# SamsungLabs/fcaf3d

Measured on AMD Instinct MI355X. Metric: scenes/sec fwd+bwd, ScanNet 100k-pt 2cm voxels, 1/2/4/8 MI355X, higher is better.
Workload: dtype f32

## Files before the change

fcaf3d_amd/csrc/conv.hip:

```cpp
#include "fc_common.h"
#include "../../include/fcaf3d_hip.h"
#ifdef FC_TRACE
__device__ unsigned long long* g_trace_buf_lds;
__device__ int g_trace_cap_lds;
extern "C" int fc_debug_trace_lds(unsigned long long* buf, int cap) {
  FC_HIP(hipMemcpyToSymbol(HIP_SYMBOL(g_trace_buf_lds), &buf, sizeof(buf)));
  FC_HIP(hipMemcpyToSymbol(HIP_SYMBOL(g_trace_cap_lds), &cap, sizeof(cap)));
  return FC_OK;
}
#define TR_BUF g_trace_buf_lds
#define TR_CAP g_trace_cap_lds
#endif
#include "fc_trace.h"

typedef float f32x16 __attribute__((ext_vector_type(16)));
typedef float f32x2 __attribute__((ext_vector_type(2)));
typedef float f32x4 __attribute__((ext_vector_type(4)));

__device__ __attribute__((aligned(16))) float g_zero_row[64];

__device__ int g_fc_prio;
extern "C" int fc_debug_set_prio(int mode) {
  FC_HIP(hipMemcpyToSymbol(HIP_SYMBOL(g_fc_prio), &mode, sizeof(mode)));
  return FC_OK;
// ... 33 lines not shown

__global__ __launch_bounds__(256) void k_amax(const f32x4* __restrict__ x, int64_t n4, const float* __restrict__ tail, int ntail,
                                              unsigned* __restrict__ slot) {
  __shared__ unsigned wm[4];
  __shared__ int last_s;
  unsigned m = 0u;
  const int64_t stride = (int64_t)gridDim.x * 256;
  for (int64_t i = (int64_t)blockIdx.x * 256 + threadIdx.x; i < n4; i += 4 * stride) {
    f32x4 v[4];
#pragma unroll
    for (int q = 0; q < 4; ++q) v[q] = i + q * stride < n4 ? x[i + q * stride] : f32x4{0.f, 0.f, 0.f, 0.f};
#pragma unroll
    for (int q = 0; q < 4; ++q)
#pragma unroll
      for (int j = 0; j < 4; ++j) { const unsigned u = __float_as_uint(v[q][j]) & 0x7fffffffu; m = (u > m && u < 0x7f800000u) ? u : m; }
  }
  if (blockIdx.x == 0 && (int)threadIdx.x < ntail) { const unsigned u = __float_as_uint(tail[threadIdx.x]) & 0x7fffffffu; m = (u > m && u < 0x7f800000u) ? u : m; }
#pragma unroll
  for (int off = 32; off > 0; off >>= 1) { const unsigned o = (unsigned)__shfl_xor((int)m, off, 64); m = o > m ? o : m; }
  if ((threadIdx.x & 63) == 0) wm[threadIdx.x >> 6] = m;
  __syncthreads();
  if (threadIdx.x == 0) {
    unsigned b = wm[0];
    for (int w = 1; w < 4; ++w) b = wm[w] > b ? wm[w] : b;
    if (b > __hip_atomic_load(&slot[1], __ATOMIC_RELAXED, __HIP_MEMORY_SCOPE_AGENT)) atomicMax(&slot[1], b);
    __threadfence();
    last_s = atomicAdd(&slot[2], 1u) == gridDim.x - 1;
    if (last_s) {
      __threadfence();
      slot[0] = atomicExch(&slot[1], 0u);
      slot[2] = 0u;
    }
  }
}

constexpr int AMAX_RING = 2048;
static unsigned* g_amax_ring[16] = {};
static unsigned g_amax_next[16] = {};
static std::mutex g_amax_ring_mu;
static int amax_ring_slot(unsigned** slot) {
  int dev = 0;
  FC_HIP(hipGetDevice(&dev));
  if (dev < 0 || dev >= 16) return FC_EINVAL;
  std::lock_guard<std::mutex> lock(g_amax_ring_mu);
  if (!g_amax_ring[dev]) {
    FC_HIP(hipMalloc((void**)&g_amax_ring[dev], (size_t)AMAX_RING * FC_AMAX_SLOT_BYTES));
    FC_HIP(hipMemset(g_amax_ring[dev], 0, (size_t)AMAX_RING * FC_AMAX_SLOT_BYTES));
  }
  const unsigned i = __atomic_fetch_add(&g_amax_next[dev], 1u, __ATOMIC_RELAXED) % AMAX_RING;
  *slot = g_amax_ring[dev] + (size_t)i * (FC_AMAX_SLOT_BYTES / 4);
  return FC_OK;
}
static int amax_launch(const float* x, int64_t n, unsigned* slot, hipStream_t stream) {
  if (n <= 0) { FC_HIP(hipMemsetAsync(slot, 0, 4, stream)); return FC_OK; }
  const int64_t n4 = n / 4;
  int64_t blocks = fc_cdiv(n4 > 0 ? n4 : 1, 256 * 8);
  if (blocks > 1024) blocks = 1024;
  k_amax<<<(unsigned)blocks, 256, 0, stream>>>(reinterpret_cast<const f32x4*>(x), n4, x + 4 * n4, (int)(n - 4 * n4), slot);
  FC_CHECK_LAUNCH();
  return FC_OK;
}
static thread_local const unsigned* t_amax_hint[2] = {nullptr, nullptr};
struct AmaxHintScope { ~AmaxHintScope() { t_amax_hint[0] = t_amax_hint[1] = nullptr; } };
static int operand_amax(const float* x, int64_t n, int which, hipStream_t stream, const unsigned** out) {
  const unsigned* h = t_amax_hint[which];
  if (h) { *out = h; return FC_OK; }
  unsigned* slot;
  int rc = amax_ring_slot(&slot);
  if (rc) return rc;
  rc = amax_launch(x, n, slot, stream);
  *out = slot;
  return rc;
}
extern "C" int fc_amax(const float* x, int64_t n, unsigned* slot, hipStream_t stream) {
  if (!slot || n < 0 || (n > 0 && !x) || ((uintptr_t)x & 15)) return FC_EINVAL;
  return amax_launch(x, n, slot, stream);
}
extern "C" int fc_conv_amax_hint(const unsigned* amax_in, const unsigned* amax_gout) {
  t_amax_hint[0] = amax_in;
  t_amax_hint[1] = amax_gout;
  return FC_OK;
}

__global__ void k_sum_parts(const float* __restrict__ part, float* __restrict__ out, int64_t elems4, int S) {
  int64_t i = (int64_t)blockIdx.x * blockDim.x + threadIdx.x;
  if (i >= elems4) return;
  float4 a = reinterpret_cast<const float4*>(part)[i];
  for (int s = 1; s < S; ++s) {
    float4 b = reinterpret_cast<const float4*>(part)[(int64_t)s * elems4 + i];
    a.x += b.x; a.y += b.y; a.z += b.z; a.w += b.w;
  }
  reinterpret_cast<float4*>(out)[i] = a;
}

__global__ void k_sum_pairs(const float* __restrict__ part, const int* __restrict__ pos, float* __restrict__ out,
                            int64_t n_out, int K, int Cout) {
  const int c4n = Cout / 4;
  int64_t t = (int64_t)blockIdx.x * blockDim.x + threadIdx.x;
  if (t >= n_out * c4n) return;
  int64_t o = t / c4n;
  int c4 = (int)(t % c4n);
  f32x4 a = {0.f, 0.f, 0.f, 0.f};
  for (int k0 = 0; k0 < K; k0 += 9) {
    int j[9];
#pragma unroll
    for (int u = 0; u < 9; ++u) j[u] = k0 + u < K ? pos[(int64_t)(k0 + u) * n_out + o] : -1;
    f32x4 v[9];
#pragma unroll
    for (int u = 0; u < 9; ++u) {
      const float* src = j[u] >= 0 ? part + ((int64_t)(k0 + u) * n_out + j[u]) * Cout + c4 * 4 : g_zero_row + (c4 & 15) * 4;
      v[u] = *reinterpret_cast<const f32x4*>(src);
    }
#pragma unroll
    for (int u = 0; u < 9; ++u)
      if (j[u] >= 0) a += v[u];
  }
  *reinterpret_cast<f32x4*>(out + o * Cout + c4 * 4) = a;
}

__host__ __device__ static inline int fc_stat_rb(int64_t n) { return n <= 1024 ? 16 : (n <= 4096 ? 64 : 32); }

__device__ __forceinline__ void stat_block_reduce(f32x4 a1, f32x4 a2, float* __restrict__ stats, int C, f32x4* sm ) {
  const int lane = threadIdx.x & 15, rl = threadIdx.x >> 4;
  sm[(rl * 2 + 0) * 16 + lane] = a1;
  sm[(rl * 2 + 1) * 16 + lane] = a2;
  __syncthreads();
  if (rl < 2) {
    f32x4 t = {0.f, 0.f, 0.f, 0.f};
#pragma unroll
    for (int q = 0; q < 16; ++q) t += sm[(q * 2 + rl) * 16 + lane];
    *reinterpret_cast<f32x4*>(stats + ((int64_t)blockIdx.x * 2 + rl) * C + blockIdx.y * 64 + lane * 4) = t;
  }
}

struct StatCh { f32x4 mu, is, ga, be; bool bwd, from_y, has_add; int act; };
__device__ __forceinline__ StatCh stat_channels(const X6Epi& epi, int c) {
  StatCh p;
  p.bwd = epi.bn_x != nullptr;
  p.act = epi.act;
  p.from_y = p.bwd && epi.bn_y != nullptr && epi.act != 0;
  p.has_add = p.bwd && epi.add != nullptr;
  p.mu = f32x4{0.f, 0.f, 0.f, 0.f}; p.is = f32x4{1.f, 1.f, 1.f, 1.f}; p.ga = p.is; p.be = p.mu;
  if (p.bwd) {
    p.mu = *reinterpret_cast<const f32x4*>(epi.mean + c);
    const f32x4 va = *reinterpret_cast<const f32x4*>(epi.var + c);
#pragma unroll
    for (int j = 0; j < 4; ++j) p.is[j] = 1.f / sqrtf(va[j] + epi.eps);
    if (epi.gamma) p.ga = *reinterpret_cast<const f32x4*>(epi.gamma + c);
    if (epi.beta) p.be = *reinterpret_cast<const f32x4*>(epi.beta + c);
  }
  return p;
}
__device__ __forceinline__ void stat_accumulate(const StatCh& p, const X6Epi& epi, const f32x4& a, int64_t at, f32x4& a1, f32x4& a2) {
  f32x4 xv = {0.f, 0.f, 0.f, 0.f}, av = xv, yv = xv;
  if (p.bwd) xv = *reinterpret_cast<const f32x4*>(epi.bn_x + at);
  if (p.has_add) av = *reinterpret_cast<const f32x4*>(epi.add + at);
  if (p.from_y) yv = *reinterpret_cast<const f32x4*>(epi.bn_y + at);
#pragma unroll
  for (int j = 0; j < 4; ++j) {
    float t1, t2;
    x6_epi_terms(p.bwd, p.bwd ? av[j] + a[j] : a[j], xv[j], p.mu[j], p.is[j], p.ga[j], p.be[j], p.act, p.from_y, yv[j], t1, t2);
    a1[j] += t1;
    a2[j] += t2;
  }
}

__global__ __launch_bounds__(256) void k_sum_parts_stats(const float* __restrict__ part, float* __restrict__ out, int64_t n, int C, int S,
                                                         int RB, X6Epi epi) {
  __shared__ f32x4 sm[16 * 2 * 16];
  const int lane = threadIdx.x & 15, rl = threadIdx.x >> 4;
  const int64_t r0 = (int64_t)blockIdx.x * RB;
  const int c = blockIdx.y * 64 + lane * 4;
  const StatCh p = stat_channels(epi, c);
  f32x4 a1 = {0.f, 0.f, 0.f, 0.f}, a2 = a1;
  for (int64_t r = r0 + rl; r < r0 + RB && r < n; r += 16) {
    f32x4 a = *reinterpret_cast<const f32x4*>(part + r * C + c);
    for (int z = 1; z < S; ++z) a += *reinterpret_cast<const f32x4*>(part + ((int64_t)z * n + r) * C + c);
    *reinterpret_cast<f32x4*>(out + r * C + c) = a;
    stat_accumulate(p, epi, a, r * C + c, a1, a2);
  }
  stat_block_reduce(a1, a2, epi.stats, C, sm);
}

__global__ __launch_bounds__(256) void k_sum_pairs_stats(const float* __restrict__ part, const int* __restrict__ pos, float* __restrict__ out,
                                                         int64_t n_out, int K, int Cout, int RB, X6Epi epi) {
  __shared__ f32x4 sm[16 * 2 * 16];
  const int lane = threadIdx.x & 15, rl = threadIdx.x >> 4;
  const int64_t r0 = (int64_t)blockIdx.x * RB;
  const int c = blockIdx.y * 64 + lane * 4;
  const StatCh p = stat_channels(epi, c);
  f32x4 a1 = {0.f, 0.f, 0.f, 0.f}, a2 = a1;
  const int64_t rend = (r0 + RB < n_out) ? r0 + RB : n_out;
  for (int64_t o = r0 + rl; o < rend; o += 32) {
    const int64_t o2 = o + 16;
    const bool two = o2 < rend;
    f32x4 a = {0.f, 0.f, 0.f, 0.f}, b = a;
    for (int k0 = 0; k0 < K; k0 += 9) {
      int j[9], j2[9];
#pragma unroll
      for (int u = 0; u < 9; ++u) {
        j[u] = k0 + u < K ? pos[(int64_t)(k0 + u) * n_out + o] : -1;
        j2[u] = (two && k0 + u < K) ? pos[(int64_t)(k0 + u) * n_out + o2] : -1;
      }
      f32x4 v[9], v2[9];
#pragma unroll
      for (int u = 0; u < 9; ++u) {
        const float* src = j[u] >= 0 ? part + ((int64_t)(k0 + u) * n_out + j[u]) * Cout + c : g_zero_row + lane * 4;
        const float* src2 = j2[u] >= 0 ? part + ((int64_t)(k0 + u) * n_out + j2[u]) * Cout + c : g_zero_row + lane * 4;
        v[u] = *reinterpret_cast<const f32x4*>(src);
        v2[u] = *reinterpret_cast<const f32x4*>(src2);
      }
#pragma unroll
      for (int u = 0; u < 9; ++u) {
        if (j[u] >= 0) a += v[u];
        if (j2[u] >= 0) b += v2[u];
      }
    }
    *reinterpret_cast<f32x4*>(out + o * Cout + c) = a;
    stat_accumulate(p, epi, a, o * Cout + c, a1, a2);
    if (two) {
      *reinterpret_cast<f32x4*>(out + o2 * Cout + c) = b;
      stat_accumulate(p, epi, b, o2 * Cout + c, a1, a2);
    }
  }
  stat_block_reduce(a1, a2, epi.stats, Cout, sm);
}

static_assert(STEM_CIN == 3 && STEM_COUT == 64 && BK == 32, "conv_route.h spells these shapes out");

struct ConvArgs {
  const float *in, *W; const int *nbr, *out_index, *cnt; float* dst;
  int64_t n_rows; int K, Cin, Cout; X6Epi epi; hipStream_t stream;
};
#define FC_LAUNCH(...) __VA_ARGS__<<<grid, 256, 0, a.stream>>>(a.in, a.W, a.nbr, a.out_index, a.cnt, a.dst, a.n_rows, a.K, a.Cin, a.Cout)
#define FC_LAUNCH_EPI(...) __VA_ARGS__<<<grid, 256, 0, a.stream>>>(a.in, a.W, a.nbr, a.out_index, a.cnt, a.dst, a.n_rows, a.K, a.Cin, a.Cout, a.epi)

template <int BM, int BN, int WM>
static void launch_conv_fp32(const ConvRoute& r, const ConvArgs& a, dim3 grid) {
#define FC_LAUNCH_MFMA(KERNEL)                                                                                              \
  do { if (r.wsrc == FC_WSRC_FP32_T) FC_LAUNCH(KERNEL<BM, BN, 32, true, WM, true>); else if (a.nbr) FC_LAUNCH(KERNEL<BM, BN, 32, true, WM>); \
       else FC_LAUNCH(KERNEL<BM, BN, 32, false, WM>); } while (0)
  if (r.family == FC_FAM_MFMA) FC_LAUNCH_MFMA(k_conv_mfma);
  if constexpr (BM >= 128) {
    if (r.family == FC_FAM_MFMA_P) FC_LAUNCH_MFMA(k_conv_mfma_p);
    if (r.family == FC_FAM_GLDS) { if (a.nbr) FC_LAUNCH(k_conv_glds<BM, BN, true, WM>); else FC_LAUNCH(k_conv_glds<BM, BN, false, WM>); }
  }
#undef FC_LAUNCH_MFMA
}

template <int BM, int BN, int WM>
static void launch_conv_x6(const ConvRoute& r, const ConvArgs& a, dim3 grid) {
  if (r.family == FC_FAM_H3R) {
    if constexpr (BM == 128) {
      if (r.buf) FC_LAUNCH_EPI(k_conv_h3r<BN, true, true>);
      else if (a.nbr) FC_LAUNCH_EPI(k_conv_h3r<BN, true, false>);
      else FC_LAUNCH_EPI(k_conv_h3r<BN, false, false>);
    }
  } else if (r.wsrc == FC_WSRC_FP32_T) FC_LAUNCH_EPI(k_conv_x6<BM, BN, true, WM, 1>);
  else if (r.wsrc == FC_WSRC_FP32) { if (a.nbr) FC_LAUNCH_EPI(k_conv_x6<BM, BN, true, WM, 0>); else FC_LAUNCH_EPI(k_conv_x6<BM, BN, false, WM, 0>); }
  else if (r.mode == FC_MODE_BF16 || r.buf) {
    if constexpr (BM == 128) {
      if (r.mode == FC_MODE_BF16) { if (a.nbr) FC_LAUNCH_EPI(k_conv_x6<128, BN, true, 2, 2, 1>); else FC_LAUNCH_EPI(k_conv_x6<128, BN, false, 2, 2, 1>); }
      else if (r.mode == FC_MODE_H3) FC_LAUNCH_EPI(k_conv_x6<128, BN, true, 2, 2, 2, true>);
      else FC_LAUNCH_EPI(k_conv_x6<128, BN, true, 2, 2, 0, true>);
    }
  } else if (r.mode == FC_MODE_H3) { if (a.nbr) FC_LAUNCH_EPI(k_conv_x6<BM, BN, true, WM, 2, 2>); else FC_LAUNCH_EPI(k_conv_x6<BM, BN, false, WM, 2, 2>); }
  else { if (a.nbr) FC_LAUNCH_EPI(k_conv_x6<BM, BN, true, WM, 2>); else FC_LAUNCH_EPI(k_conv_x6<BM, BN, false, WM, 2>); }
}

static int launch_conv(const ConvRoute& r, const ConvArgs& a) {
  const dim3 grid(r.grid[0], r.grid[1], r.grid[2]);
  if (r.family == FC_FAM_STEM) {
    const size_t smem = (size_t)(STEM_ROWS * STEM_FWD_LDA + 96 * 64) * sizeof(float);
    k_stem_fwd<<<(unsigned)fc_cdiv(a.n_rows, STEM_ROWS), 256, smem, a.stream>>>(a.in, a.W, a.nbr, a.dst, nullptr, a.n_rows, a.K);
  } else if (r.family == FC_FAM_FMA) {
    k_conv_fma<<<(unsigned)fc_cdiv(a.n_rows * a.Cout, 256), 256, 0, a.stream>>>(a.in, a.W, a.nbr, a.dst, a.n_rows, a.K, a.Cin, a.Cout, r.wsrc == FC_WSRC_FP32_T ? 1 : 0);
  } else {
#define FC_TILE(BM, BN, WM) do { if (r.family >= FC_FAM_X6) launch_conv_x6<BM, BN, WM>(r, a, grid); else launch_conv_fp32<BM, BN, WM>(r, a, grid); } while (0)
    if (r.bm == 256) FC_TILE(256, 64, 4);
    else if (r.bm == 128 && r.bn == 128) FC_TILE(128, 128, 2);
    else if (r.bm == 128) FC_TILE(128, 64, 2);
    else if (r.bn == 128) launch_conv_fp32<64, 128, 2>(r, a, grid);
    else launch_conv_fp32<64, 64, 2>(r, a, grid);
#undef FC_TILE
  }
  FC_CHECK_LAUNCH();
  return FC_OK;
}
#undef FC_LAUNCH
#undef FC_LAUNCH_EPI

extern "C" {

int fc_conv_fwd_route(int64_t n_in, int64_t n_out, int K, int Cin, int Cout, int flags, int table_kind, int64_t live_tiles, int* out) {
  if (!out || n_in < 0 || n_out < 0 || K < 1 || Cin < 1 || Cout < 1) return FC_EINVAL;
  const ConvRoute r = conv_route({n_in, n_out, K, Cin, Cout}, flags, table_kind, live_tiles, route_env());
  const int f[16] = {r.family, r.bm, r.bn, r.wm, r.S, r.wsrc, r.mode, r.buf, r.epi, (int)r.grid[0], (int)r.grid[1], (int)r.grid[2]};
  for (int i = 0; i < 16; ++i) out[i] = f[i];
  return r.family == FC_FAM_INVALID ? FC_EINVAL : FC_OK;
}

int64_t fc_conv_fwd_ws_bytes(int64_t n_out, int K, int Cin, int Cout, int flags) {
  const ConvRoute r = conv_route({n_out, n_out, K, Cin, Cout}, flags, FC_TABLE_DENSE, 0, route_env());
  return r.S > 1 ? (int64_t)r.S * n_out * Cout * (int64_t)sizeof(float) : 0;
}

int64_t fc_conv_fwd_pairs_ws_bytes(int64_t n_out, int K, int Cout) {
  return (int64_t)K * n_out * Cout * (int64_t)sizeof(float);
}

int64_t fc_conv_stats_blocks(int64_t n_out, int K, int Cin, int Cout, int flags, int pairs) {
  if (n_out < 1) return 0;
  const ConvRoute r = conv_route({n_out, n_out, K, Cin, Cout}, flags, pairs ? FC_TABLE_PAIRS : FC_TABLE_DENSE, 0, route_env());
  if (r.epi == FC_EPI_NONE) return 0;
  return r.epi == FC_EPI_SUM ? fc_cdiv(n_out, fc_stat_rb(n_out)) : fc_cdiv(n_out, r.bm);
}

static int conv_impl(const float* in, const float* W, const int* nbr, const int* out_index, const int* cnt, const int* pos, float* out,
                     int64_t n_in, int64_t n_out, int K, int Cin, int Cout, int64_t live_tiles, int flags, void* ws, int64_t ws_bytes,
                     hipStream_t stream, const X6Epi* epi) {
  AmaxHintScope hint_scope;
  if (n_in < 0 || n_out < 0 || K < 1 || Cin < 1 || Cout < 1) return FC_EINVAL;
  if (n_out == 0 && !cnt) return epi ? FC_EINVAL : FC_OK;
  if (out_index && !nbr) return FC_EINVAL;
  const int table = cnt ? FC_TABLE_PAIRS : out_index ? FC_TABLE_SORTED : nbr ? FC_TABLE_DENSE : FC_TABLE_NONE;
  const ConvRoute r = conv_route({n_in, n_out, K, Cin, Cout}, flags, table | (epi ? FC_TABLE_STATS : 0), live_tiles, route_env());
  if (r.family == FC_FAM_INVALID) return FC_EINVAL;
  if (n_out == 0) return FC_OK;
  ConvArgs a = {in, W, nbr, out_index, cnt, out, n_out, K, Cin, Cout, {}, stream};
  if (r.family == FC_FAM_STEM || r.family == FC_FAM_FMA) return launch_conv(r, a);
  const bool parts = cnt || r.S > 1;
  if (parts && ws_bytes < (int64_t)r.S * n_out * Cout * (int64_t)sizeof(float)) return FC_EWS;
  if (parts) a.dst = (float*)ws;
  if (epi && r.epi == FC_EPI_KERNEL) a.epi = *epi;
  int rc = FC_OK;
  if (r.mode == FC_MODE_H3) rc = operand_amax(in, n_in * (int64_t)Cin, 0, stream, &a.epi.amax_in);
  if (rc == FC_OK) rc = launch_conv(r, a);
  if (rc != FC_OK || !parts) return rc;
  const int rb = fc_stat_rb(n_out);
  const dim3 sgrid((unsigned)fc_cdiv(n_out, rb), Cout / 64);
  if (cnt && epi) k_sum_pairs_stats<<<sgrid, 256, 0, stream>>>(a.dst, pos, out, n_out, K, Cout, rb, *epi);
  else if (cnt) k_sum_pairs<<<(unsigned)fc_cdiv(n_out * (Cout / 4), 256), 256, 0, stream>>>(a.dst, pos, out, n_out, K, Cout);
  else if (epi) k_sum_parts_stats<<<sgrid, 256, 0, stream>>>(a.dst, out, n_out, Cout, r.S, rb, *epi);
  else k_sum_parts<<<(unsigned)fc_cdiv(n_out * Cout / 4, 256), 256, 0, stream>>>(a.dst, out, n_out * Cout / 4, r.S);
  FC_CHECK_LAUNCH();
  return FC_OK;
}

static int conv_pairs_impl(const float* in, const float* W, const int* pair_in, const int* pair_cnt, const int* pair_pos, float* out,
                           int64_t n_in, int64_t n_out, int K, int Cin, int Cout, int64_t live_tiles, int flags, void* ws,
                           int64_t ws_bytes, hipStream_t stream, const X6Epi* epi) {
  if (!pair_in || !pair_cnt || !pair_pos || K > 65535) return FC_EINVAL;
  return conv_impl(in, W, pair_in, nullptr, pair_cnt, pair_pos, out, n_in, n_out, K, Cin, Cout, live_tiles, flags, ws, ws_bytes, stream, epi);
}

static X6Epi stats_epi(float* stats, const float* bn_x = nullptr, const float* mean = nullptr, const float* var = nullptr, const float* gamma = nullptr,
                       const float* beta = nullptr, float eps = 0.f, int act = 0, const float* add = nullptr, const float* bn_y = nullptr) {
  return {stats, bn_x, mean, var, gamma, beta, eps, act, add, bn_y, nullptr};
}

int fc_conv_fwd(const float* in, const float* W, const int* nbr, const int* out_index, float* out, int64_t n_in,
                int64_t n_out, int K, int Cin, int Cout, int flags, void* ws, int64_t ws_bytes, hipStream_t stream) {
  return conv_impl(in, W, nbr, out_index, nullptr, nullptr, out, n_in, n_out, K, Cin, Cout, 0, flags, ws, ws_bytes, stream, nullptr);
}

int fc_conv_fwd_stats(const float* in, const float* W, const int* nbr, const int* out_index, float* out, int64_t n_in,
                      int64_t n_out, int K, int Cin, int Cout, int flags, void* ws, int64_t ws_bytes, float* stats,
                      hipStream_t stream) {
  const X6Epi e = stats_epi(stats);
  return conv_impl(in, W, nbr, out_index, nullptr, nullptr, out, n_in, n_out, K, Cin, Cout, 0, flags, ws, ws_bytes, stream, stats ? &e : nullptr);
}

int fc_conv_fwd_bn_bwd_stats(const float* in, const float* W, const int* nbr, const int* out_index, float* out, int64_t n_in,
                             int64_t n_out, int K, int Cin, int Cout, int flags, void* ws, int64_t ws_bytes, float* stats,
                             const float* bn_x, const float* mean, const float* var, const float* gamma, const float* beta, float eps,
                             int act, const float* add, const float* bn_y, hipStream_t stream) {
  if (!stats || !bn_x || !mean || !var || act < 0 || act > 2) return FC_EINVAL;
  const X6Epi e = stats_epi(stats, bn_x, mean, var, gamma, beta, eps, act, add, bn_y);
  return conv_impl(in, W, nbr, out_index, nullptr, nullptr, out, n_in, n_out, K, Cin, Cout, 0, flags, ws, ws_bytes, stream, &e);
}

int fc_conv_fwd_pairs_tiles(const float* in, const float* W, const int* pair_in, const int* pair_cnt, const int* pair_pos,
                            float* out, int64_t n_in, int64_t n_out, int K, int Cin, int Cout, int64_t live_tiles, int flags,
                            void* ws, int64_t ws_bytes, hipStream_t stream) {
  return conv_pairs_impl(in, W, pair_in, pair_cnt, pair_pos, out, n_in, n_out, K, Cin, Cout, live_tiles, flags, ws, ws_bytes, stream, nullptr);
}

int fc_conv_fwd_pairs_tiles_stats(const float* in, const float* W, const int* pair_in, const int* pair_cnt, const int* pair_pos,
                                  float* out, int64_t n_in, int64_t n_out, int K, int Cin, int Cout, int64_t live_tiles, int flags,
                                  void* ws, int64_t ws_bytes, float* stats, hipStream_t stream) {
  const X6Epi e = stats_epi(stats);
  return conv_pairs_impl(in, W, pair_in, pair_cnt, pair_pos, out, n_in, n_out, K, Cin, Cout, live_tiles, flags, ws, ws_bytes, stream,
                         stats ? &e : nullptr);
}

int fc_conv_fwd_pairs_tiles_bn_bwd_stats(const float* in, const float* W, const int* pair_in, const int* pair_cnt, const int* pair_pos,
                                         float* out, int64_t n_in, int64_t n_out, int K, int Cin, int Cout, int64_t live_tiles, int flags,
                                         void* ws, int64_t ws_bytes, float* stats, const float* bn_x, const float* mean,
                                         const float* var, const float* gamma, const float* beta, float eps, int act,
                                         const float* add, const float* bn_y, hipStream_t stream) {
  if (!stats || !bn_x || !mean || !var || act < 0 || act > 2) return FC_EINVAL;
  const X6Epi e = stats_epi(stats, bn_x, mean, var, gamma, beta, eps, act, add, bn_y);
  return conv_pairs_impl(in, W, pair_in, pair_cnt, pair_pos, out, n_in, n_out, K, Cin, Cout, live_tiles, flags, ws, ws_bytes, stream, &e);
}

int fc_conv_fwd_pairs(const float* in, const float* W, const int* pair_in, const int* pair_cnt, const int* pair_pos,
                      float* out, int64_t n_in, int64_t n_out, int K, int Cin, int Cout, int flags, void* ws,
                      int64_t ws_bytes, hipStream_t stream) {
  return fc_conv_fwd_pairs_tiles(in, W, pair_in, pair_cnt, pair_pos, out, n_in, n_out, K, Cin, Cout, 0, flags, ws, ws_bytes, stream);
}

int64_t fc_x6_weight_image_bytes(int K, int R, int C) { return (int64_t)K * R * C * 6; }

int fc_x6_weight_image(const float* W, void* img, int K, int R, int C, int transposed, hipStream_t stream) {
  if (K < 1 || R < 32 || C < 64 || R % 32 != 0 || C % 64 != 0) return FC_EINVAL;
  const int64_t total = (int64_t)K * (R / 32) * (C / 64) * 256;
  const unsigned nb = (unsigned)fc_cdiv(total, 256);
  if (split_mode() == 2) {
    FC_HIP(hipMemsetAsync((char*)img + 4 * X6_IMG_AMAX_WORD, 0, FC_AMAX_SLOT_BYTES, stream));
    k_x6_weight_image<3><<<nb, 256, 0, stream>>>(W, (u32x4*)img, K, R, C, transposed);
    k_x6_weight_image<2><<<nb, 256, 0, stream>>>(W, (u32x4*)img, K, R, C, transposed);
  } else {
    k_x6_weight_image<0><<<nb, 256, 0, stream>>>(W, (u32x4*)img, K, R, C, transposed);
  }
  FC_CHECK_LAUNCH();
  return FC_OK;
}
// ... 235 lines not shown
```

fcaf3d_amd/csrc/norm_bn.h:

```cpp
#pragma once


__global__ void k_bn1_partial(const float* __restrict__ x, int64_t n, int C, int64_t rpb, float* __restrict__ part) {
  extern __shared__ float sm[];
  const auto [cl, rl, nrl] = lane_coord(C / 4);
  const auto [r0, r1] = row_span(rpb, n);
  const float4 sh = *reinterpret_cast<const float4*>(x + cl * 4);
  float4 a1 = make_float4(0.f, 0.f, 0.f, 0.f), a2 = a1;
  for (int64_t rb = r0 + rl; rb < r1; rb += 4 * (int64_t)nrl) {
    float4 v[4];
#pragma unroll
    for (int u = 0; u < 4; ++u) {
      const int64_t r = rb + (int64_t)u * nrl;
      v[u] = *reinterpret_cast<const float4*>(x + (r < r1 ? r : 0) * C + cl * 4);
    }
#pragma unroll
    for (int u = 0; u < 4; ++u) {
      v[u].x -= sh.x; v[u].y -= sh.y; v[u].z -= sh.z; v[u].w -= sh.w;
      a1.x += v[u].x; a1.y += v[u].y; a1.z += v[u].z; a1.w += v[u].w;
      a2.x += v[u].x * v[u].x; a2.y += v[u].y * v[u].y; a2.z += v[u].z * v[u].z; a2.w += v[u].w * v[u].w;
    }
  }
  *reinterpret_cast<float4*>(&sm[(rl * 2 + 0) * C + cl * 4]) = a1;
  *reinterpret_cast<float4*>(&sm[(rl * 2 + 1) * C + cl * 4]) = a2;
// ... 151 lines not shown
                                unsigned* __restrict__ amax_out) {
  extern __shared__ float sm[];
  const int c0 = blockIdx.y * CG;
  x += c0; gy += c0; gx += c0; mean += c0; var += c0;
  if (y) y += c0;
  if (gy2) gy2 += c0;
  if (gres) gres += c0;
  if (gamma) gamma += c0;
  if (beta) beta += c0;
  const int c4n = CG / 4;
  const int cl = threadIdx.x % c4n, rl = threadIdx.x / c4n;
  const int nrl = blockDim.x / c4n;
  float4 t1, t2;
  bn1_reduce_parts(part, nb, C, cl, rl, nrl, sm, &t1, &t2, CG, c0);
  if (blockIdx.x == 0 && rl == 0) {
    *reinterpret_cast<float4*>(sums + c0 + cl * 4) = t1;
    *reinterpret_cast<float4*>(sums + C + c0 + cl * 4) = t2;
  }
  const float inv_n = 1.f / (float)n;
  float s1[4] = {t1.x * inv_n, t1.y * inv_n, t1.z * inv_n, t1.w * inv_n};
  float s2[4] = {t2.x * inv_n, t2.y * inv_n, t2.z * inv_n, t2.w * inv_n};
  float mu[4], is[4], g[4], bt[4];
#pragma unroll
  for (int j = 0; j < 4; ++j) {
    mu[j] = mean[cl * 4 + j];
    is[j] = 1.f / sqrtf(var[cl * 4 + j] + eps);
    g[j] = gamma ? gamma[cl * 4 + j] : 1.f;
    bt[j] = beta ? beta[cl * 4 + j] : 0.f;
  }
  const bool from_y = act && y;
  const auto [r0, r1] = row_span(rpb, n);
  unsigned am = 0u;
  for (int64_t rb = r0 + rl; rb < r1; rb += 4 * (int64_t)nrl) {
    float xv[4][4], gv[4][4], yv[4][4];
#pragma unroll
    for (int u = 0; u < 4; ++u) {
      const int64_t r = rb + (int64_t)u * nrl;
      const int64_t rc = r < r1 ? r : r0;
      *reinterpret_cast<float4*>(xv[u]) = *reinterpret_cast<const float4*>(x + rc * C + cl * 4);
      *reinterpret_cast<float4*>(gv[u]) = *reinterpret_cast<const float4*>(gy + rc * C + cl * 4);
      if (gy2) {
        const float4 t2 = *reinterpret_cast<const float4*>(gy2 + rc * C + cl * 4);
        gv[u][0] += t2.x; gv[u][1] += t2.y; gv[u][2] += t2.z; gv[u][3] += t2.w;
      }
      if (from_y) *reinterpret_cast<float4*>(yv[u]) = *reinterpret_cast<const float4*>(y + rc * C + cl * 4);
    }
#pragma unroll
    for (int u = 0; u < 4; ++u) {
      const int64_t r = rb + (int64_t)u * nrl;
      if (r >= r1) continue;
      float o[4], gr[4];
#pragma unroll
      for (int j = 0; j < 4; ++j) {
        float gg = gv[u][j];
        if (from_y) gg *= act_bwd_from_y(yv[u][j], act);
        else if (act) gg *= act_bwd_from_pre(bn_pre(xv[u][j], mu[j], is[j], g[j], bt[j]), act);
        float xh = (xv[u][j] - mu[j]) * is[j];
        gr[j] = gg;
        o[j] = g[j] * is[j] * (gg - s1[j] - xh * s2[j]);
      }
      *reinterpret_cast<float4*>(gx + r * C + cl * 4) = *reinterpret_cast<float4*>(o);
      if (gres) *reinterpret_cast<float4*>(gres + r * C + cl * 4) = *reinterpret_cast<float4*>(gr);
#pragma unroll
      for (int j = 0; j < 4; ++j) amax_fold(am, o[j]);
    }
  }
  if (amax_out) amax_commit(am, amax_out);
}

__global__ void k_bn2_apply(const float* __restrict__ x, int64_t n, int C, int64_t rpb, const float* __restrict__ part, int nb, int G,
                            float eps, const float* __restrict__ gamma, const float* __restrict__ beta,
                            const float* __restrict__ residual, int act, float momentum, float* __restrict__ y,
                            float* __restrict__ mean_out, float* __restrict__ var_out, float* __restrict__ cnt_out,
                            float* __restrict__ rmean, float* __restrict__ rvar, long long* __restrict__ nbt, int CG,
                            const int* __restrict__ add_inv, const float* __restrict__ add_src, unsigned* __restrict__ amax_out) {
  extern __shared__ double smd[];
  const int c0 = blockIdx.y * CG;
  x += c0; y += c0; part += c0; mean_out += c0; var_out += c0;
  if (add_src) add_src += c0;
  if (residual) residual += c0;
  if (gamma) gamma += c0;
  if (beta) beta += c0;
  if (rmean) { rmean += c0; rvar += c0; }
  const auto [cl, rl, nrl] = lane_coord(CG / 4);
  double a1[4] = {0., 0., 0., 0.}, a2[4] = {0., 0., 0., 0.};
  const int GC = G * C;
  for (int t = rl; t < nb * G; t += nrl) {
    const int b = t / G, g = t % G;
    const float* src = part + ((int64_t)b * 2) * GC + g * C + cl * 4;
    const float4 u = fc_ld4(src), w = fc_ld4(src + GC);
    a1[0] += u.x; a1[1] += u.y; a1[2] += u.z; a1[3] += u.w;
    a2[0] += w.x; a2[1] += w.y; a2[2] += w.z; a2[3] += w.w;
  }
#pragma unroll
  for (int j = 0; j < 4; ++j) {
    smd[(rl * 2 + 0) * CG + cl * 4 + j] = a1[j];
    smd[(rl * 2 + 1) * CG + cl * 4 + j] = a2[j];
  }
  __syncthreads();
  float mu[4], va[4], is[4], g[4], bt[4];
#pragma unroll
  for (int j = 0; j < 4; ++j) {
    double t1 = 0., t2 = 0.;
    for (int q = 0; q < nrl; ++q) { t1 += smd[(q * 2 + 0) * CG + cl * 4 + j]; t2 += smd[(q * 2 + 1) * CG + cl * 4 + j]; }
    bn2_stats(t1, t2, n, &mu[j], &va[j]);
    is[j] = 1.f / sqrtf(va[j] + eps);
    g[j] = gamma ? gamma[cl * 4 + j] : 1.f;
    bt[j] = beta ? beta[cl * 4 + j] : 0.f;
  }
  if (blockIdx.x == 0 && rl == 0) {
    *reinterpret_cast<float4*>(mean_out + cl * 4) = make_float4(mu[0], mu[1], mu[2], mu[3]);
    *reinterpret_cast<float4*>(var_out + cl * 4) = make_float4(va[0], va[1], va[2], va[3]);
    if (cl == 0 && blockIdx.y == 0) { cnt_out[0] = (float)n; if (nbt) nbt[0] += 1; }
    if (rmean) {
#pragma unroll
      for (int j = 0; j < 4; ++j) bn_running_update(rmean, rvar, cl * 4 + j, mu[j], va[j], (float)n, momentum);
    }
  }
  const auto [r0, r1] = row_span(rpb, n);
  unsigned am = 0u;
  for (int64_t rb = r0 + rl; rb < r1; rb += 4 * (int64_t)nrl) {
    float v[4][4], rs[4][4];
    int q[4];
#pragma unroll
    for (int u = 0; u < 4; ++u) {
      const int64_t r = rb + (int64_t)u * nrl;
      const int64_t rc = r < r1 ? r : r0;
      *reinterpret_cast<float4*>(v[u]) = *reinterpret_cast<const float4*>(x + rc * C + cl * 4);
      if (residual) *reinterpret_cast<float4*>(rs[u]) = *reinterpret_cast<const float4*>(residual + rc * C + cl * 4);
      q[u] = add_inv ? add_inv[rc] : -1;
    }
#pragma unroll
    for (int u = 0; u < 4; ++u) {
      const int64_t r = rb + (int64_t)u * nrl;
      if (r >= r1) continue;
      float o[4];
#pragma unroll
      for (int j = 0; j < 4; ++j) o[j] = norm_act_elem(v[u][j], mu[j], is[j], g[j], bt[j], residual ? &rs[u][j] : nullptr, act);
      if (q[u] >= 0) {
        const float4 f = *reinterpret_cast<const float4*>(add_src + (int64_t)q[u] * C + cl * 4);
        o[0] += f.x; o[1] += f.y; o[2] += f.z; o[3] += f.w;
      }
      *reinterpret_cast<float4*>(y + r * C + cl * 4) = *reinterpret_cast<float4*>(o);
#pragma unroll
      for (int j = 0; j < 4; ++j) amax_fold(am, o[j]);
    }
  }
  if (amax_out) amax_commit(am, amax_out);
}

__global__ __launch_bounds__(256) void k_bn2_finalize(const float* __restrict__ part, int nb, int C, int G, int64_t n, float momentum,
                                                       float* __restrict__ mean, float* __restrict__ var, float* __restrict__ cnt,
                                                       float* __restrict__ rmean, float* __restrict__ rvar,
                                                       long long* __restrict__ nbt) {
  __shared__ double r1[FIN_SL][FIN_CB + 1], r2[FIN_SL][FIN_CB + 1];
  const int cl = threadIdx.x & (FIN_CB - 1), j = threadIdx.x / FIN_CB;
  const int c = blockIdx.x * FIN_CB + cl;
  const int GC = G * C;
  double a1 = 0., a2 = 0.;
  if (c < C) {
    double p1[4] = {0., 0., 0., 0.}, p2[4] = {0., 0., 0., 0.};
    const int total = nb * G;
    int t = j;
    for (; t + 3 * FIN_SL < total; t += 4 * FIN_SL) {
      float u[4], w[4];
#pragma unroll
      for (int q = 0; q < 4; ++q) {
        const int tt = t + FIN_SL * q, b = tt / G, g = tt % G;
        u[q] = fc_ld(&part[((int64_t)b * 2) * GC + g * C + c]);
        w[q] = fc_ld(&part[((int64_t)b * 2 + 1) * GC + g * C + c]);
      }
#pragma unroll
      for (int q = 0; q < 4; ++q) { p1[q] += u[q]; p2[q] += w[q]; }
    }
    for (; t < total; t += FIN_SL) {
      const int b = t / G, g = t % G;
      p1[0] += fc_ld(&part[((int64_t)b * 2) * GC + g * C + c]);
      p2[0] += fc_ld(&part[((int64_t)b * 2 + 1) * GC + g * C + c]);
    }
    a1 = (p1[0] + p1[1]) + (p1[2] + p1[3]);
    a2 = (p2[0] + p2[1]) + (p2[2] + p2[3]);
  }
  r1[j][cl] = a1;
  r2[j][cl] = a2;
  __syncthreads();
  if (j == 0 && c < C) {
    double s1 = 0., s2 = 0.;
    for (int q = 0; q < FIN_SL; ++q) { s1 += r1[q][cl]; s2 += r2[q][cl]; }
    float mu, va;
    bn2_stats(s1, s2, n, &mu, &va);
    mean[c] = mu;
    var[c] = va;
    if (c == 0) { cnt[0] = (float)n; if (nbt) nbt[0] += 1; }
    if (rmean) bn_running_update(rmean, rvar, c, mu, va, (float)n, momentum);
  }
}

extern "C" __global__ void k_bn_running(const float* __restrict__ mean, const float* __restrict__ var, const float* __restrict__ cnt,
                             float momentum, int C, float* __restrict__ rmean, float* __restrict__ rvar,
                             long long* __restrict__ nbt) {
  int c = blockIdx.x * blockDim.x + threadIdx.x;
  if (c == 0 && nbt) nbt[0] += 1;
  if (c >= C) return;
  float n = cnt[0];
  float unbias = n / fmaxf(n - 1.f, 1.f);
  rmean[c] = (1.f - momentum) * rmean[c] + momentum * mean[c];
  rvar[c] = (1.f - momentum) * rvar[c] + momentum * var[c] * unbias;
}
```

Baseline: 523.5.

## Batch partial-sum loads and prefetch BN rows ahead of stat reduction

The split-K partial-sum kernels now process a fixed number of rows per thread and issue batched independent loads across slices or kernel offsets. The pair kernel loads position indices once per lane and broadcasts them with shuffles. Stat operands are loaded before the summation so their latency overlaps it, and the rsqrt is deferred. In the BN apply kernel, the first rows of x/residual are requested before the partial-stat reduction and barrier, and the partial loop is unrolled four-wide to expose memory-level parallelism. The cost is higher register pressure and more template instantiations.

```diff
diff --git a/fcaf3d_amd/csrc/conv.hip b/fcaf3d_amd/csrc/conv.hip
--- a/fcaf3d_amd/csrc/conv.hip
+++ b/fcaf3d_amd/csrc/conv.hip
@@ -139,6 +139,31 @@
   return FC_OK;
 }
 
+constexpr int SUM_LOADS = 36, SUM_PAIR_LOADS = 24;
+static inline int sum_parts_zb(int nr, int S) {
+  const int cap = SUM_LOADS / nr >= 27 ? 27 : SUM_LOADS / nr;
+  return S <= 3 ? 3 : (S <= 9 || cap == 9) ? 9 : (S <= 18 || cap == 18) ? 18 : 27;
+}
+
+template <int NR, int ZB>
+__device__ __forceinline__ void sum_parts_chunk(const float* __restrict__ part, const int64_t (&at)[NR], int64_t slab, int z0, int S, f32x4 (&a)[NR]) {
+  f32x4 v[NR][ZB];
+#pragma unroll
+  for (int u = 0; u < ZB; ++u) {
+    const int z = z0 + u < S ? z0 + u : S - 1;
+#pragma unroll
+    for (int i = 0; i < NR; ++i) v[i][u] = *reinterpret_cast<const f32x4*>(part + (int64_t)z * slab + at[i]);
+  }
+#pragma unroll
+  for (int u = 0; u < ZB; ++u) {
+#pragma unroll
+    for (int i = 0; i < NR; ++i) {
+      if (z0 + u == 0) a[i] = v[i][u];
+      else if (z0 + u < S) a[i] += v[i][u];
+    }
+  }
+}
+
 __global__ void k_sum_parts(const float* __restrict__ part, float* __restrict__ out, int64_t elems4, int S) {
   int64_t i = (int64_t)blockIdx.x * blockDim.x + threadIdx.x;
   if (i >= elems4) return;
@@ -148,6 +173,74 @@
     a.x += b.x; a.y += b.y; a.z += b.z; a.w += b.w;
   }
   reinterpret_cast<float4*>(out)[i] = a;
+}
+
+constexpr int SUM_KC = 27;
+struct PosWords { int w[2]; };
+__device__ __forceinline__ PosWords pos_words(const int* __restrict__ pos, int64_t n_out, int64_t o , bool live, int kc, int K, int lane) {
+  PosWords p;
+#pragma unroll
+  for (int h = 0; h < 2; ++h) {
+    const int k = kc + 16 * h + lane;
+    const int j = pos[(int64_t)(k < K ? k : K - 1) * n_out + o];
+    p.w[h] = (live && k < K && 16 * h + lane < SUM_KC) ? j : -1;
+  }
+  return p;
+}
+__device__ __forceinline__ int pos_word(const PosWords& p, int u) { return __shfl(p.w[u >> 4], u & 15, 16); }
+
+template <int NR, int KB>
+__device__ __forceinline__ void sum_pairs_batch(const float* __restrict__ part, const PosWords (&w)[NR], int64_t n_out, int Cout, int c, int zc,
+                                                int kc, int kb, int K, f32x4 (&a)[NR]) {
+  int j[NR][KB];
+  f32x4 v[NR][KB];
+#pragma unroll
+  for (int u = 0; u < KB; ++u) {
+#pragma unroll
+    for (int i = 0; i < NR; ++i) {
+      j[i][u] = kb + u < SUM_KC ? pos_word(w[i], kb + u) : -1;
+      v[i][u] = f32x4{0.f, 0.f, 0.f, 0.f};
+    }
+  }
+#pragma unroll
+  for (int g = 0; g < KB; g += 9) {
+    if (kc + kb + g < K) {
+#pragma unroll
+      for (int u = g; u < g + 9 && u < KB; ++u) {
+#pragma unroll
+        for (int i = 0; i < NR; ++i) {
+          const float* src = j[i][u] >= 0 ? part + ((int64_t)(kc + kb + u) * n_out + j[i][u]) * Cout + c : g_zero_row + zc;
+          v[i][u] = *reinterpret_cast<const f32x4*>(src);
+        }
+      }
+    }
+  }
+#pragma unroll
+  for (int u = 0; u < KB; ++u) {
+#pragma unroll
+    for (int i = 0; i < NR; ++i)
+      if (j[i][u] >= 0) a[i] += v[i][u];
+  }
+}
+template <int NR, int KB, int KB0>
+__device__ __forceinline__ void sum_pairs_batches(const float* __restrict__ part, const PosWords (&w)[NR], int64_t n_out, int Cout, int c, int zc, int kc,
+                                                  int K, f32x4 (&a)[NR]) {
+  if constexpr (KB0 < SUM_KC) {
+    if (kc + KB0 < K) sum_pairs_batch<NR, (KB < SUM_KC - KB0 ? KB : SUM_KC - KB0)>(part, w, n_out, Cout, c, zc, kc, KB0, K, a);
+    sum_pairs_batches<NR, KB, KB0 + KB>(part, w, n_out, Cout, c, zc, kc, K, a);
+  }
+}
+template <int NR>
+__device__ __forceinline__ void sum_pairs_rows(const float* __restrict__ part, const int* __restrict__ pos, PosWords (&w)[NR], const int64_t (&o)[NR],
+                                               const bool (&live)[NR], int64_t n_out, int K, int Cout, int c, int lane, f32x4 (&a)[NR]) {
+  constexpr int KB = SUM_PAIR_LOADS / NR;
+  for (int kc = 0; kc < K; kc += SUM_KC) {
+    sum_pairs_batches<NR, KB, 0>(part, w, n_out, Cout, c, lane * 4, kc, K, a);
+    if (kc + SUM_KC < K) {
+#pragma unroll
+      for (int i = 0; i < NR; ++i) w[i] = pos_words(pos, n_out, o[i], live[i], kc + SUM_KC, K, lane);
+    }
+  }
 }
 
 __global__ void k_sum_pairs(const float* __restrict__ part, const int* __restrict__ pos, float* __restrict__ out,
@@ -191,8 +284,10 @@
 }
 
 struct StatCh { f32x4 mu, is, ga, be; bool bwd, from_y, has_add; int act; };
-__device__ __forceinline__ StatCh stat_channels(const X6Epi& epi, int c) {
-  StatCh p;
+struct StatChRaw { StatCh p; };
+__device__ __forceinline__ StatChRaw stat_channel_loads(const X6Epi& epi, int c) {
+  StatChRaw r;
+  StatCh& p = r.p;
   p.bwd = epi.bn_x != nullptr;
   p.act = epi.act;
   p.from_y = p.bwd && epi.bn_y != nullptr && epi.act != 0;
@@ -200,87 +295,124 @@
   p.mu = f32x4{0.f, 0.f, 0.f, 0.f}; p.is = f32x4{1.f, 1.f, 1.f, 1.f}; p.ga = p.is; p.be = p.mu;
   if (p.bwd) {
     p.mu = *reinterpret_cast<const f32x4*>(epi.mean + c);
-    const f32x4 va = *reinterpret_cast<const f32x4*>(epi.var + c);
-#pragma unroll
-    for (int j = 0; j < 4; ++j) p.is[j] = 1.f / sqrtf(va[j] + epi.eps);
+    p.is = *reinterpret_cast<const f32x4*>(epi.var + c);
     if (epi.gamma) p.ga = *reinterpret_cast<const f32x4*>(epi.gamma + c);
     if (epi.beta) p.be = *reinterpret_cast<const f32x4*>(epi.beta + c);
   }
+  return r;
+}
+__device__ __forceinline__ StatCh stat_channels(const StatChRaw& r, float eps) {
+  StatCh p = r.p;
+  if (p.bwd) {
+#pragma unroll
+    for (int j = 0; j < 4; ++j) p.is[j] = 1.f / sqrtf(p.is[j] + eps);
+  }
   return p;
 }
-__device__ __forceinline__ void stat_accumulate(const StatCh& p, const X6Epi& epi, const f32x4& a, int64_t at, f32x4& a1, f32x4& a2) {
-  f32x4 xv = {0.f, 0.f, 0.f, 0.f}, av = xv, yv = xv;
-  if (p.bwd) xv = *reinterpret_cast<const f32x4*>(epi.bn_x + at);
-  if (p.has_add) av = *reinterpret_cast<const f32x4*>(epi.add + at);
-  if (p.from_y) yv = *reinterpret_cast<const f32x4*>(epi.bn_y + at);
+struct StatOps { f32x4 xv, av, yv; };
+__device__ __forceinline__ StatOps stat_operands(const StatCh& p, const X6Epi& epi, int64_t at) {
+  StatOps q;
+  q.xv = f32x4{0.f, 0.f, 0.f, 0.f}; q.av = q.xv; q.yv = q.xv;
+  if (p.bwd) q.xv = *reinterpret_cast<const f32x4*>(epi.bn_x + at);
+  if (p.has_add) q.av = *reinterpret_cast<const f32x4*>(epi.add + at);
+  if (p.from_y) q.yv = *reinterpret_cast<const f32x4*>(epi.bn_y + at);
+  return q;
+}
+__device__ __forceinline__ void stat_accumulate(const StatCh& p, const StatOps& q, const f32x4& a, f32x4& a1, f32x4& a2) {
 #pragma unroll
   for (int j = 0; j < 4; ++j) {
     float t1, t2;
-    x6_epi_terms(p.bwd, p.bwd ? av[j] + a[j] : a[j], xv[j], p.mu[j], p.is[j], p.ga[j], p.be[j], p.act, p.from_y, yv[j], t1, t2);
+    x6_epi_terms(p.bwd, p.bwd ? q.av[j] + a[j] : a[j], q.xv[j], p.mu[j], p.is[j], p.ga[j], p.be[j], p.act, p.from_y, q.yv[j], t1, t2);
     a1[j] += t1;
     a2[j] += t2;
   }
 }
 
-__global__ __launch_bounds__(256) void k_sum_parts_stats(const float* __restrict__ part, float* __restrict__ out, int64_t n, int C, int S,
-                                                         int RB, X6Epi epi) {
+template <int NR>
+struct SumRows {
+  int lane, rl, c;
+  int64_t o[NR];
+  bool live[NR];
+  __device__ __forceinline__ SumRows(int64_t n) {
+    lane = threadIdx.x & 15, rl = threadIdx.x >> 4, c = blockIdx.y * 64 + lane * 4;
+#pragma unroll
+    for (int i = 0; i < NR; ++i) {
+      const int64_t r = (int64_t)blockIdx.x * (NR * 16) + rl + 16 * i;
+      live[i] = r < n;
+      o[i] = live[i] ? r : n - 1;
+    }
+  }
+};
+template <int NR>
+__device__ __forceinline__ void sum_rows_finish(const SumRows<NR>& t, const StatCh& p, const StatOps (&q)[NR], const f32x4 (&a)[NR], float* __restrict__ out,
+                                                float* __restrict__ stats, int C, f32x4* sm) {
+  f32x4 a1 = {0.f, 0.f, 0.f, 0.f}, a2 = a1;
+#pragma unroll
+  for (int i = 0; i < NR; ++i) {
+    if (t.live[i]) {
+      *reinterpret_cast<f32x4*>(out + t.o[i] * C + t.c) = a[i];
+      stat_accumulate(p, q[i], a[i], a1, a2);
+    }
+  }
+  stat_block_reduce(a1, a2, stats, C, sm);
+}
+
+template <int NR, int ZB>
+__global__ __launch_bounds__(256) void k_sum_parts_stats(const float* __restrict__ part, float* __restrict__ out, int64_t n, int C, int S, X6Epi epi) {
   __shared__ f32x4 sm[16 * 2 * 16];
-  const int lane = threadIdx.x & 15, rl = threadIdx.x >> 4;
-  const int64_t r0 = (int64_t)blockIdx.x * RB;
-  const int c = blockIdx.y * 64 + lane * 4;
-  const StatCh p = stat_channels(epi, c);
-  f32x4 a1 = {0.f, 0.f, 0.f, 0.f}, a2 = a1;
-  for (int64_t r = r0 + rl; r < r0 + RB && r < n; r += 16) {
-    f32x4 a = *reinterpret_cast<const f32x4*>(part + r * C + c);
-    for (int z = 1; z < S; ++z) a += *reinterpret_cast<const f32x4*>(part + ((int64_t)z * n + r) * C + c);
-    *reinterpret_cast<f32x4*>(out + r * C + c) = a;
-    stat_accumulate(p, epi, a, r * C + c, a1, a2);
-  }
-  stat_block_reduce(a1, a2, epi.stats, C, sm);
-}
-
+  const SumRows<NR> t(n);
+  const StatChRaw pr = stat_channel_loads(epi, t.c);
+  int64_t at[NR];
+  StatOps q[NR];
+  f32x4 a[NR];
+#pragma unroll
+  for (int i = 0; i < NR; ++i) {
+    at[i] = t.o[i] * C + t.c;
+    q[i] = stat_operands(pr.p, epi, at[i]);
+  }
+  for (int z0 = 0; z0 < S; z0 += ZB) sum_parts_chunk<NR, ZB>(part, at, n * C, z0, S, a);
+  sum_rows_finish<NR>(t, stat_channels(pr, epi.eps), q, a, out, epi.stats, C, sm);
+}
+
+template <int NR>
 __global__ __launch_bounds__(256) void k_sum_pairs_stats(const float* __restrict__ part, const int* __restrict__ pos, float* __restrict__ out,
-                                                         int64_t n_out, int K, int Cout, int RB, X6Epi epi) {
+                                                         int64_t n_out, int K, int Cout, X6Epi epi) {
   __shared__ f32x4 sm[16 * 2 * 16];
-  const int lane = threadIdx.x & 15, rl = threadIdx.x >> 4;
-  const int64_t r0 = (int64_t)blockIdx.x * RB;
-  const int c = blockIdx.y * 64 + lane * 4;
-  const StatCh p = stat_channels(epi, c);
-  f32x4 a1 = {0.f, 0.f, 0.f, 0.f}, a2 = a1;
-  const int64_t rend = (r0 + RB < n_out) ? r0 + RB : n_out;
-  for (int64_t o = r0 + rl; o < rend; o += 32) {
-    const int64_t o2 = o + 16;
-    const bool two = o2 < rend;
-    f32x4 a = {0.f, 0.f, 0.f, 0.f}, b = a;
-    for (int k0 = 0; k0 < K; k0 += 9) {
-      int j[9], j2[9];
-#pragma unroll
-      for (int u = 0; u < 9; ++u) {
-        j[u] = k0 + u < K ? pos[(int64_t)(k0 + u) * n_out + o] : -1;
-        j2[u] = (two && k0 + u < K) ? pos[(int64_t)(k0 + u) * n_out + o2] : -1;
-      }
-      f32x4 v[9], v2[9];
-#pragma unroll
-      for (int u = 0; u < 9; ++u) {
-        const float* src = j[u] >= 0 ? part + ((int64_t)(k0 + u) * n_out + j[u]) * Cout + c : g_zero_row + lane * 4;
-        const float* src2 = j2[u] >= 0 ? part + ((int64_t)(k0 + u) * n_out + j2[u]) * Cout + c : g_zero_row + lane * 4;
-        v[u] = *reinterpret_cast<const f32x4*>(src);
-        v2[u] = *reinterpret_cast<const f32x4*>(src2);
-      }
-#pragma unroll
-      for (int u = 0; u < 9; ++u) {
-        if (j[u] >= 0) a += v[u];
-        if (j2[u] >= 0) b += v2[u];
-      }
-    }
-    *reinterpret_cast<f32x4*>(out + o * Cout + c) = a;
-    stat_accumulate(p, epi, a, o * Cout + c, a1, a2);
-    if (two) {
-      *reinterpret_cast<f32x4*>(out + o2 * Cout + c) = b;
-      stat_accumulate(p, epi, b, o2 * Cout + c, a1, a2);
-    }
-  }
-  stat_block_reduce(a1, a2, epi.stats, Cout, sm);
+  const SumRows<NR> t(n_out);
+  PosWords w[NR];
+#pragma unroll
+  for (int i = 0; i < NR; ++i) w[i] = pos_words(pos, n_out, t.o[i], t.live[i], 0, K, t.lane);
+  const StatChRaw pr = stat_channel_loads(epi, t.c);
+  StatOps q[NR];
+  f32x4 a[NR];
+#pragma unroll
+  for (int i = 0; i < NR; ++i) {
+    q[i] = stat_operands(pr.p, epi, t.o[i] * Cout + t.c);
+    a[i] = f32x4{0.f, 0.f, 0.f, 0.f};
+  }
+  sum_pairs_rows<NR>(part, pos, w, t.o, t.live, n_out, K, Cout, t.c, t.lane, a);
+  sum_rows_finish<NR>(t, stat_channels(pr, epi.eps), q, a, out, epi.stats, Cout, sm);
+}
+
+static void launch_sum(const float* part, const int* pos, float* out, int64_t n_out, int K, int Cout, int S, const X6Epi* epi, hipStream_t stream) {
+  const int rb = fc_stat_rb(n_out), nr = rb / 16;
+  const dim3 sgrid((unsigned)fc_cdiv(n_out, rb), Cout / 64);
+  const int zb = sum_parts_zb(nr, S);
+  if (pos && epi) {
+    if (nr == 1) k_sum_pairs_stats<1><<<sgrid, 256, 0, stream>>>(part, pos, out, n_out, K, Cout, *epi);
+    else if (nr == 2) k_sum_pairs_stats<2><<<sgrid, 256, 0, stream>>>(part, pos, out, n_out, K, Cout, *epi);
+    else k_sum_pairs_stats<4><<<sgrid, 256, 0, stream>>>(part, pos, out, n_out, K, Cout, *epi);
+  } else if (pos) {
+    k_sum_pairs<<<(unsigned)fc_cdiv(n_out * (Cout / 4), 256), 256, 0, stream>>>(part, pos, out, n_out, K, Cout);
+  } else if (epi) {
+#define FC_SUM_PARTS(NR, ZB) k_sum_parts_stats<NR, ZB><<<sgrid, 256, 0, stream>>>(part, out, n_out, Cout, S, *epi)
+    if (nr == 1) { if (zb == 3) FC_SUM_PARTS(1, 3); else if (zb == 9) FC_SUM_PARTS(1, 9); else if (zb == 18) FC_SUM_PARTS(1, 18); else FC_SUM_PARTS(1, 27); }
+    else if (nr == 2) { if (zb == 3) FC_SUM_PARTS(2, 3); else if (zb == 9) FC_SUM_PARTS(2, 9); else FC_SUM_PARTS(2, 18); }
+    else { if (zb == 3) FC_SUM_PARTS(4, 3); else FC_SUM_PARTS(4, 9); }
+#undef FC_SUM_PARTS
+  } else {
+    k_sum_parts<<<(unsigned)fc_cdiv(n_out * Cout / 4, 256), 256, 0, stream>>>(part, out, n_out * Cout / 4, S);
+  }
 }
 
 static_assert(STEM_CIN == 3 && STEM_COUT == 64 && BK == 32, "conv_route.h spells these shapes out");
@@ -394,12 +526,7 @@
   if (r.mode == FC_MODE_H3) rc = operand_amax(in, n_in * (int64_t)Cin, 0, stream, &a.epi.amax_in);
   if (rc == FC_OK) rc = launch_conv(r, a);
   if (rc != FC_OK || !parts) return rc;
-  const int rb = fc_stat_rb(n_out);
-  const dim3 sgrid((unsigned)fc_cdiv(n_out, rb), Cout / 64);
-  if (cnt && epi) k_sum_pairs_stats<<<sgrid, 256, 0, stream>>>(a.dst, pos, out, n_out, K, Cout, rb, *epi);
-  else if (cnt) k_sum_pairs<<<(unsigned)fc_cdiv(n_out * (Cout / 4), 256), 256, 0, stream>>>(a.dst, pos, out, n_out, K, Cout);
-  else if (epi) k_sum_parts_stats<<<sgrid, 256, 0, stream>>>(a.dst, out, n_out, Cout, r.S, rb, *epi);
-  else k_sum_parts<<<(unsigned)fc_cdiv(n_out * Cout / 4, 256), 256, 0, stream>>>(a.dst, out, n_out * Cout / 4, r.S);
+  launch_sum(a.dst, cnt ? pos : nullptr, out, n_out, K, Cout, r.S, epi, stream);
   FC_CHECK_LAUNCH();
   return FC_OK;
 }
diff --git a/fcaf3d_amd/csrc/norm_bn.h b/fcaf3d_amd/csrc/norm_bn.h
--- a/fcaf3d_amd/csrc/norm_bn.h
+++ b/fcaf3d_amd/csrc/norm_bn.h
@@ -257,15 +257,47 @@
   if (gamma) gamma += c0;
   if (beta) beta += c0;
   if (rmean) { rmean += c0; rvar += c0; }
-  const auto [cl, rl, nrl] = lane_coord(CG / 4);
+  const LaneCoord lc = lane_coord(CG / 4);
+  const int cl = lc.cl, rl = lc.rl, nrl = lc.nrl;
+  const RowSpan span = row_span(rpb, n);
+  const int64_t r0 = span.r0, r1 = span.r1;
+  float v[4][4], rs[4][4];
+  int q[4];
+  auto request_rows = [&](int64_t rb) {
+#pragma unroll
+    for (int u = 0; u < 4; ++u) {
+      const int64_t r = rb + (int64_t)u * nrl;
+      const int64_t rc = r < r1 ? r : r0;
+      *reinterpret_cast<float4*>(v[u]) = *reinterpret_cast<const float4*>(x + rc * C + cl * 4);
+      if (residual) *reinterpret_cast<float4*>(rs[u]) = *reinterpret_cast<const float4*>(residual + rc * C + cl * 4);
+      q[u] = add_inv ? add_inv[rc] : -1;
+    }
+  };
+  if (r0 < r1) request_rows(r0 + rl);
+  float g[4], bt[4];
+#pragma unroll
+  for (int j = 0; j < 4; ++j) {
+    g[j] = gamma ? gamma[cl * 4 + j] : 1.f;
+    bt[j] = beta ? beta[cl * 4 + j] : 0.f;
+  }
   double a1[4] = {0., 0., 0., 0.}, a2[4] = {0., 0., 0., 0.};
-  const int GC = G * C;
-  for (int t = rl; t < nb * G; t += nrl) {
-    const int b = t / G, g = t % G;
-    const float* src = part + ((int64_t)b * 2) * GC + g * C + cl * 4;
-    const float4 u = fc_ld4(src), w = fc_ld4(src + GC);
-    a1[0] += u.x; a1[1] += u.y; a1[2] += u.z; a1[3] += u.w;
-    a2[0] += w.x; a2[1] += w.y; a2[2] += w.z; a2[3] += w.w;
+  const int GC = G * C, nt = nb * G;
+  for (int t0 = rl; t0 < nt; t0 += 4 * nrl) {
+    float4 u[4], w[4];
+#pragma unroll
+    for (int i = 0; i < 4; ++i) {
+      const int t = t0 + i * nrl < nt ? t0 + i * nrl : 0;
+      const int b = t / G, g = t % G;
+      const float* src = part + ((int64_t)b * 2) * GC + g * C + cl * 4;
+      u[i] = fc_ld4(src), w[i] = fc_ld4(src + GC);
+    }
+#pragma unroll
+    for (int i = 0; i < 4; ++i) {
+      if (t0 + i * nrl < nt) {
+        a1[0] += u[i].x; a1[1] += u[i].y; a1[2] += u[i].z; a1[3] += u[i].w;
+        a2[0] += w[i].x; a2[1] += w[i].y; a2[2] += w[i].z; a2[3] += w[i].w;
+      }
+    }
   }
 #pragma unroll
   for (int j = 0; j < 4; ++j) {
@@ -273,15 +305,13 @@
     smd[(rl * 2 + 1) * CG + cl * 4 + j] = a2[j];
   }
   __syncthreads();
-  float mu[4], va[4], is[4], g[4], bt[4];
+  float mu[4], va[4], is[4];
 #pragma unroll
   for (int j = 0; j < 4; ++j) {
     double t1 = 0., t2 = 0.;
     for (int q = 0; q < nrl; ++q) { t1 += smd[(q * 2 + 0) * CG + cl * 4 + j]; t2 += smd[(q * 2 + 1) * CG + cl * 4 + j]; }
     bn2_stats(t1, t2, n, &mu[j], &va[j]);
     is[j] = 1.f / sqrtf(va[j] + eps);
-    g[j] = gamma ? gamma[cl * 4 + j] : 1.f;
-    bt[j] = beta ? beta[cl * 4 + j] : 0.f;
   }
   if (blockIdx.x == 0 && rl == 0) {
     *reinterpret_cast<float4*>(mean_out + cl * 4) = make_float4(mu[0], mu[1], mu[2], mu[3]);
@@ -292,19 +322,9 @@
       for (int j = 0; j < 4; ++j) bn_running_update(rmean, rvar, cl * 4 + j, mu[j], va[j], (float)n, momentum);
     }
   }
-  const auto [r0, r1] = row_span(rpb, n);
   unsigned am = 0u;
   for (int64_t rb = r0 + rl; rb < r1; rb += 4 * (int64_t)nrl) {
-    float v[4][4], rs[4][4];
-    int q[4];
-#pragma unroll
-    for (int u = 0; u < 4; ++u) {
-      const int64_t r = rb + (int64_t)u * nrl;
-      const int64_t rc = r < r1 ? r : r0;
-      *reinterpret_cast<float4*>(v[u]) = *reinterpret_cast<const float4*>(x + rc * C + cl * 4);
-      if (residual) *reinterpret_cast<float4*>(rs[u]) = *reinterpret_cast<const float4*>(residual + rc * C + cl * 4);
-      q[u] = add_inv ? add_inv[rc] : -1;
-    }
+    if (rb != r0 + rl) request_rows(rb);
 #pragma unroll
     for (int u = 0; u < 4; ++u) {
       const int64_t r = rb + (int64_t)u * nrl;
```

Result: no change. 524.3, median of 2 (+0.2%).
